# Linux-cpp-lisp/sitator

Measured on AMD Instinct MI355X. Metric: landmark-vectors/sec (frames x mobile atoms), fill + site assignment, higher is better.
Workload: dtype f64; 1 GPU; C2: SCgrid(8,8,8) orthorhombic 32.0x35.2x38.4 A, S=D=512 (V=8), M=64, A=576 (BASELINE configs[1]), 100000 frames per GPU; frames_per_gpu=100000, n_mobile=64, n_static=512, landmark_dim=512, parallelism=frame-sharded x1

## Files before the change

scratch/phase_times.py:

```python
import os, sys
sys.path.insert(0, os.path.dirname(os.path.dirname(os.path.abspath(__file__))))
os.environ["SITATOR_FILL_AUTOTUNE"] = "0"
import numpy as np
from tests.test_gpu_kernels import _setup
from sitator_amd import synth
cfg = sys.argv[1] if len(sys.argv) > 1 else "C2"
F = int(sys.argv[2]) if len(sys.argv) > 2 else 100000
host = synth.config_host(cfg)
ctx, *_ = _setup(host, synth.CONFIG_MOBILE[cfg], F, seed=2)
for _ in range(30):
    ctx.fill(check_for_zeros=False)
out = {}
for mode in (11, 10, 12):
    os.environ["SITATOR_DEBUG_STOP"] = str(mode)
    for _ in range(3):
        rc, nz, err = ctx.fill(check_for_zeros=False)
    out[mode] = ctx.info()["census"]
    print("mode", mode, "fill ms %.4f" % ctx.timers()["fill"], out[mode])
os.environ.pop("SITATOR_DEBUG_STOP")
nw = out[11][3]
names = {10: ["start -> barrier A passed", "A -> barrier B passed (phase 1b)", "B -> window set-up done", "D0 passes"],
         11: ["D1 + E passes", "T + end of window", "whole wave", None],
         12: ["start -> frame requested, at barrier A", "wait at barrier A", "phase 1b work", "wait at barrier B"]}
print("waves %d; shader-clock cycles per wave (s_memtime, 100 MHz ticks x clock ratio = cycles as the SQ counts them):" % nw)
for mode in (10, 11, 12):
    for n, v in zip(names[mode], out[mode]):
        if n:
            print("  %-44s %9.0f" % (n, v / nw))
```

sitator_amd/csrc/fill3.hip:

```cpp
#include <cmath>
#include <cstdio>
#include <cstdlib>
#include <mutex>
#include <vector>
#include <algorithm>
#include <cstring>

#include "sit_internal.h"
#include "fill3_plan.h"

struct Fill3Args {
    const uint4 *vh;
    const uint4 *vh16;
    const unsigned char *nvtab;
    const uint4 *pack;
    const i32 *p_off, *f_off;
    const i32 *lattice_map;
    i32 *row_nnz, *row_idx;
    double *row_val;
    i64 N;
    int D, W;
    int pG0, pG1, pG2, fG0, fG1, fG2;
    unsigned f_base;
    int check_zeros;
    double midpoint, steepness;
    u64 *err, *scal;
    i64 frame0;
    double cen[3];
    double x0lo, x0hi;
    int nv_uniform;
    u64 *dbgbuf;
    const i32 *static_idx, *mobile_idx;
    const double *frame_dmax;
    int s0, m0, frame_mod;
    double delta2, thr2_lo, thr2_hi, static_thr;
    int store;
    const i32 *col_ptr, *col_k;
    const double *col_val;
    i64 *labels;
    double *confs;
    i32 *wlist;
    unsigned *wcount;
    i64 seg_cap;
    int nseg, normed;
    double threshold;
};

struct Fill3Head {
    Pbc P;
    const double *frames;
    const double *ref_static;
    const double *exptab;
    i64 F, A, fbeg;
    int S, M, fpb, contig, debug_stop, rcap, iw, has_fallback, tt, mcap, prio;
    int skipw;
    int lay[12];
    double safe2;
};
typedef const Fill3Args __attribute__((address_space(4))) *Fill3ArgsPtr;


__device__ __forceinline__ double sqrt_nr(double x)
{
    const double y = __builtin_amdgcn_rsq(x);
    const double g = x * y, h = 0.5 * y;
    const double r = __builtin_fma(-h, g, 0.5);
    return __builtin_fma(g, r, g);
}

__device__ __forceinline__ double rcp_nr(double b)
{
    double y = __builtin_amdgcn_rcp(b);
    double e = __builtin_fma(-b, y, 1.0);
    y = __builtin_fma(y, e, y);
    e = __builtin_fma(-b, y, 1.0);
    return __builtin_fma(y, e, y);
}

struct ExpK {
    double log2e_128, magic, ln2_128, c4, c3, smid;
};
__device__ __forceinline__ double in_vgpr(double x) { asm volatile("" : "+v"(x)); return x; }
__device__ __forceinline__ double max_f64(double x, double c)
{
    double r;
    asm("v_max_f64 %0, %1, %2" : "=v"(r) : "v"(x), "s"(c));
    return r;
}
__device__ __forceinline__ ExpK expk_make(double mid, double steep)
{
    ExpK k;
    k.log2e_128 = in_vgpr(0x1.71547652b82fep+7);
    k.magic = in_vgpr(6755399441055744.0);
    k.ln2_128 = in_vgpr(0x1.62e42fefa39efp-8);
    k.c4 = in_vgpr(1.0 / 24); k.c3 = in_vgpr(1.0 / 6);
    k.smid = in_vgpr(steep * mid);
    return k;
}

__device__ __forceinline__ double exp_tab(double x, const double *tab, const ExpK &k)
{
    x = max_f64(x, -700.0);
    double u;
    asm("v_fma_f64 %0, %1, %2, %3" : "=v"(u) : "v"(x), "v"(k.log2e_128), "v"(k.magic));
    const double n = u - k.magic;
    const int ni = (int)(unsigned)__double_as_longlong(u);
    const double r = __builtin_fma(-n, k.ln2_128, x);
    double q = __builtin_fma(r, k.c4, k.c3);
    q = __builtin_fma(r, q, 0.5);
// ... 79 lines not shown

#define F3_LANES(m) __builtin_amdgcn_inverse_ballot_w64(m)

__device__ __forceinline__ unsigned long long first_lanes(int n)
{
    return n >= 64 ? ~0ull : ((1ull << n) - 1ull);
}

template <int CELL>
__device__ __forceinline__ void wrapc3(const Pbc &P, double &x, double &y, double &z)
{
    if (CELL == 1) {
        double b0 = P.ci[0] * x; b0 -= floor(b0);
        double b1 = P.ci[4] * y; b1 -= floor(b1);
        double b2 = P.ci[8] * z; b2 -= floor(b2);
        x = P.cm[0] * b0; y = P.cm[4] * b1; z = P.cm[8] * b2;
    } else {
        wrap3(P, x, y, z);
    }
}

template <int CELL>
__device__ __forceinline__ int bin_of3(const Pbc &P, double px, double py, double pz, int G0, int G1, int G2)
{
    double f0, f1, f2;
    if (CELL == 1) { f0 = P.ci[0] * px; f1 = P.ci[4] * py; f2 = P.ci[8] * pz; }
    else {
        f0 = (P.ci[0] * px + P.ci[1] * py + P.ci[2] * pz);
        f1 = (P.ci[3] * px + P.ci[4] * py + P.ci[5] * pz);
        f2 = (P.ci[6] * px + P.ci[7] * py + P.ci[8] * pz);
    }
    f0 -= floor(f0); f1 -= floor(f1); f2 -= floor(f2);
    int b0 = (int)(f0 * G0), b1 = (int)(f1 * G1), b2 = (int)(f2 * G2);
    b0 = b0 < 0 ? 0 : (b0 >= G0 ? G0 - 1 : b0);
    b1 = b1 < 0 ? 0 : (b1 >= G1 ? G1 - 1 : b1);
    b2 = b2 < 0 ? 0 : (b2 >= G2 ? G2 - 1 : b2);
    return (b0 * G1 + b1) * G2 + b2;
}

#define F3_TASK_OFFSETS(TK, R0X, R0Y, VOFF, IONOFF, STATOFF, FLX)                                                          \
    do {                                                                                                                   \
        VOFF = (R0X); STATOFF = 0u; FLX = 0u;                                                                              \
        const unsigned ion_ = (TK) & ~KMASK;                                                                               \
        if (FPB1) {                                                                                                        \
            IONOFF = mad24_24(ion_, ionbase);                                                                              \
            if (DYN) VOFF = 24u * (unsigned)g.lattice_map[f0 * S + (i64)(R0Y)];                                            \
        } else {                                                                                                           \
            const uint4 ir = ((const uint4 *)ionrec)[ion_];                                                                \
            IONOFF = ir.y; STATOFF = ir.z; FLX = ir.w;                                                                     \
            if (DYN) VOFF = 24u * (unsigned)g.lattice_map[(f0 + (i64)ir.w) * S + (i64)(R0Y)];                              \
        }                                                                                                                  \
    } while (0)

#define F3_D0_PASSES(NP0)                                                                                                   \
    do {                                                                                                                    \
        uint4 en_[NP0];                                                                                                     \
        unsigned ionoff_[NP0], statoff_[NP0], tfl_[NP0];                                                                    \
        int ion_[NP0];                                                                                                      \
        unsigned long long vmask_[NP0];                                                                                     \
        uint2 ii_[NP0];                                                                                                     \
        bool in_[NP0];                                                                                                      \
        if (SLOT) {                                                                                                         \
             \
             \
                                            \
            _Pragma("unroll") for (int u = 0; u < NP0; u++) {                                                               \
                ion_[u] = base + d0_step * u + s_ion;                                                                       \
                in_[u] = ion_[u] < nib;                                                                                     \
                ii_[u] = ioninfo[ib0 + ion_[u]];                                                                            \
                ionoff_[u] = ionbase + 24u * (unsigned)(base + d0_step * u) + s_ioff;                                       \
            }                                                                                                               \
                     \
            _Pragma("unroll") for (int u = 0; u < NP0; u++) asm volatile("" : "+v"(ii_[u].x), "+v"(ii_[u].y));              \
        }                                                                                                                   \
        _Pragma("unroll") for (int u = 0; u < NP0; u++) {                                                                   \
            statoff_[u] = 0u; tfl_[u] = 0u;                                                                                 \
            if (SLOT) {                                                                                                     \
                 \
                 \
                const bool act_ = in_[u] && s_slot < (int)(ii_[u].y & 255u);                                                \
                vmask_[u] = __ballot(act_);                                                                                 \
                en_[u] = pack[act_ ? ii_[u].x + (unsigned)s_slot : 0u];                                                     \
            } else {                                                                                                        \
                en_[u] = make_uint4(0u, 0u, 0u, 0x7ff00000u);       \
                const int b_ = base + 64 * u, t = b_ + lane;                                                                \
                vmask_[u] = first_lanes(nlt0 - b_);                                                                         \
                const uint2 mw = *(const uint2 *)(mark + (b_ >> 5));                        \
                const unsigned m_lo = (unsigned)__builtin_amdgcn_readfirstlane((int)mw.x), m_hi = (unsigned)__builtin_amdgcn_readfirstlane((int)mw.y); \
                const unsigned rk = __builtin_amdgcn_mbcnt_hi(m_hi, __builtin_amdgcn_mbcnt_lo(m_lo, (unsigned)carry));      \
                carry += __builtin_popcount(m_lo) + __builtin_popcount(m_hi);                                               \
                if (FPB1) {                                                                                                 \
                    const uint2 rr = ((const uint2 *)ionrec)[rk];                                                           \
                    ion_[u] = (int)rr.y;                                                                                    \
                    if (F3_LANES(vmask_[u])) en_[u] = pack[rr.x + (unsigned)t];                                             \
                    ionoff_[u] = ionbase + 24u * (unsigned)ion_[u];                                                         \
                } else {                                                                                                    \
                    ion_[u] = (int)rk2ion[rk];                                                                              \
                    const uint4 ir = ((const uint4 *)ionrec)[ion_[u]];                                                      \
                    if (F3_LANES(vmask_[u])) en_[u] = pack[ir.x + (unsigned)t];                                             \
                    ionoff_[u] = ir.y; statoff_[u] = ir.z; tfl_[u] = ir.w;                                                  \
                }                                                                                                           \
            }                                                                                                               \
        }                                                                                                                   \
              \
        if (SLOT) { _Pragma("unroll") for (int u = 0; u < NP0; u++) asm volatile("" : "+v"(en_[u].x)); }                    \
        _Pragma("unroll") for (int u = 0; u < NP0; u++) {                                                                  \
            const uint4 en = en_[u];                                                                                       \
            unsigned voff = en.y;                                                                                          \
            if (DYN) voff = 24u * (unsigned)g.lattice_map[(f0 + (i64)tfl_[u]) * S + (i64)(en.y / 24u)];                    \
            const double hk = __hiloint2double((int)en.w, (int)en.z);                                                      \
            const double *sp = lds_f64(statoff_[u] + voff);                                                                \
            const double *op = lds_f64(ionoff_[u]);                                                                        \
            double qx = sp[0] + op[0], qy = sp[1] + op[1], qz = sp[2] + op[2];                                             \
            double d2;                                                                                                     \
            if (CHEAP) {                                                                                                   \
                       \
                                                           \
                qx = minimg1(qx, P.ci[0], P.cm[0]); qy = minimg1(qy, P.ci[4], P.cm[4]); qz = minimg1(qz, P.ci[8], P.cm[8]); \
                d2 = __builtin_fma(qz, qz, __builtin_fma(qy, qy, qx * qx));                                                \
            } else {                                                                                                       \
                wrapc3<CELL>(P, qx, qy, qz);                                                                               \
                const double dx = qx - P.cen[0], dy = qy - P.cen[1], dz = qz - P.cen[2];                                   \
                d2 = (dx * dx + dy * dy) + dz * dz;                                                                        \
            }                                                                                                              \
            const unsigned long long km = __ballot(!(d2 > hk)) & vmask_[u];                                                \
            if (F3_LANES(km)) ttab[mask_rank(km, t_end)] = (en.x & KMASK) | (unsigned)ion_[u];                             \
            t_end += __popcll(km);                                                                                         \
        }                                                                                                                  \
    } while (0)

#define F3_D1E_LOAD(NP, C0, TK, R0, CLAMP)                                                                                 \
    do {                                                                                                                   \
        _Pragma("unroll") for (int u = 0; u < NP; u++) {                                                                   \
            int tb_ = TPP * ((C0) + u);                                                                                    \
            if (CLAMP) tb_ = tb_ < TT - TPP ? tb_ : TT - TPP;                                           \
// ... 158 lines not shown
        if (act && !wsp && n >= 1 && n <= 4) {                                                                             \
            i32 d0 = (i32)(svq[0] >> KSH), d1 = 0, d2 = 0, d3 = 0;                                                         \
            double v0 = pq[0], v1 = 0.0, v2 = 0.0, v3 = 0.0;                                                               \
            if (n > 1) { d1 = (i32)(svq[1] >> KSH); v1 = pq[1]; }                                                          \
            if (n > 2) { d2 = (i32)(svq[2] >> KSH); v2 = pq[2]; }                                                          \
            if (n > 3) { d3 = (i32)(svq[3] >> KSH); v3 = pq[3]; }                                                          \
            double x2 = 0.0;                                                                                               \
            x2 += v0 * v0;                                                                                                 \
            if (n > 1) x2 += v1 * v1;                                                                                      \
            if (n > 2) x2 += v2 * v2;                                                                                      \
            if (n > 3) x2 += v3 * v3;                                                                                      \
            const double xn = sqrt(x2);                                                                                    \
            const Best b = merge4_row(n, d0, d1, d2, d3, v0, v1, v2, v3, xn, g.normed != 0, g.col_ptr, g.col_k, g.col_val); \
            i64 to;                                                                                                        \
            double conf;                                                                                                   \
            finish_assignment(b, g.threshold, to, conf);                                                                   \
            g.labels[row] = to;                                                                                            \
            g.confs[row] = conf;                                                                                           \
        }                                                                                                                  \
        if (act && !wsp && n > 4 && !g.store) {                                                                            \
            for (int e = 0; e < n; e++) {                                                                                  \
                if (e < g.W) { g.row_idx[(i64)e * g.N + row] = (i32)(svq[e] >> KSH); g.row_val[(i64)e * g.N + row] = pq[e]; } \
                else atomicAdd(&g.scal[3], 1ull);                                                                          \
            }                                                                                                              \
            g.row_nnz[row] = n < g.W ? n : g.W;                                                                            \
        }                                                                                                                  \
        const bool listed = act && n >= 1 && (wsp || n > 4);                                                               \
        if (__ballot(listed)) {                                                                                            \
            const i64 sg = (i64)(blockIdx.x % (unsigned)g.nseg);                                                           \
            list_rows_by_class(listed && n <= 8, listed && n > 8, row, g.wlist + sg * g.seg_cap, g.wcount + 2 * sg,        \
                               g.seg_cap, lane);                                                                           \
        }                                                                                                                  \
    } while (0)

template <int N>
__device__ __forceinline__ double dpp_row_shl(double x)
{
    const int lo = __double2loint(x), hi = __double2hiint(x);
    return __hiloint2double(__builtin_amdgcn_mov_dpp(hi, 0x100 + N, 0xf, 0xf, true),
                            __builtin_amdgcn_mov_dpp(lo, 0x100 + N, 0xf, 0xf, true));
}

#define F3_STAMP(var) do { if (DBG == 2 && dbg >= 10) var = __builtin_amdgcn_s_memtime(); } while (0)
#define F3_SPAN(mode, word, t0, t1) do { if (DBG == 2 && dbg == (mode) && lane == 0) atomicAdd(&g.dbgbuf[4 * (blockIdx.x & 1023u) + (word)], (u64)((t1) - (t0))); } while (0)

#ifndef F3_WPE
#define F3_WPE 7
#endif
#if F3_WPE > 0
#define F3_WPE_ATTR __attribute__((amdgpu_waves_per_eu(NW == 16 ? 8 : F3_WPE, NW == 16 ? 8 : F3_WPE)))
#else
#define F3_WPE_ATTR
#endif
template <int CELL, int LG, int NW, int DYN, int FPB1, int DBG, int FUSE, int SLOT = 0>
__global__ __launch_bounds__(NW * 64) F3_WPE_ATTR void k_fill3(Fill3Head h, Fill3ArgsPtr full)
{
    static_assert(!SLOT || FPB1, "the slot form is for one frame per workgroup");
    constexpr int VP = 1 << LG;
    constexpr bool CHEAP = CELL == 1;
    constexpr int NT = NW * 64;
    constexpr int TPP = 64 >> LG;
    constexpr int KSH = CELL == 1 ? LG + 4 : LG + 5;
    constexpr int RSH = KSH - LG;
    constexpr unsigned KMASK = ~((1u << KSH) - 1u);
    constexpr unsigned long long LEADS = LG == 4 ? 0x0001000100010001ull : (LG == 3 ? 0x0101010101010101ull : 0x1111111111111111ull);
    extern __shared__ __attribute__((aligned(16))) char smem[];
    const int S = h.S, M = h.M, SM = S + M;
    const int fpb = FPB1 ? 1 : h.fpb;
    const int tid = threadIdx.x, lane = tid & 63, wave = __builtin_amdgcn_readfirstlane(tid >> 6);
    const int rcap = h.rcap, IW = h.iw, TT = h.tt;
    const int dbg = DBG ? h.debug_stop : 0;
    F3Layout L;
    L.fmax = h.lay[0]; L.gsync = h.lay[1]; L.ioninfo = h.lay[2]; L.etab = h.lay[3]; L.wave0 = h.lay[4]; L.o_ionrec = h.lay[5];
    L.o_ttab = h.lay[6]; L.o_sv = h.lay[7]; L.o_nzc = h.lay[8]; L.o_mark = h.lay[9]; L.wbytes = h.lay[10]; L.total = h.lay[11];
    double *xyz = (double *)smem;
    u64 *fmax = (u64 *)(smem + L.fmax);
    unsigned *wflag = (unsigned *)(fmax + fpb);
    unsigned *garrive = (unsigned *)(smem + L.gsync);
    unsigned *wspill = garrive + NW;
    uint2 *ioninfo = (uint2 *)(smem + L.ioninfo);
    double *etab = (double *)(smem + L.etab);
    char *wp = smem + L.wave0 + wave * L.wbytes;
    double *prod = (double *)wp;
    unsigned *ionrec = (unsigned *)(wp + L.o_ionrec);
    unsigned *ttab = (unsigned *)(wp + L.o_ttab);
    unsigned *sv = (unsigned *)(wp + L.o_sv);
    unsigned *nzc = (unsigned *)(wp + L.o_nzc);
    unsigned *mark = (unsigned *)(wp + L.o_mark);
    unsigned char *rk2ion = (unsigned char *)(wp + L.o_ionrec) + 16 * IW;
    const Pbc &P = h.P;
    const i64 f0 = h.fbeg + (i64)blockIdx.x * fpb;
    const int nf = FPB1 ? 1 : (int)((h.F - f0) < fpb ? (h.F - f0) : fpb);
    const u64 errw = (u64)(S + 1 + M);
    const Fill3Args __attribute__((address_space(4))) &g = *full;

    if ((unsigned)(size_t)(__attribute__((address_space(3))) char *)smem != 0u) {
        if (tid == 0) atomicMin(g.err, 0ull);
        return;
    }
    unsigned long long ts0 = 0, ts1 = 0, ts2 = 0, ts3 = 0, ts4 = 0, tsa = 0, tsb = 0, acc_d0 = 0, acc_d1 = 0;
    F3_STAMP(ts0);
    const int prio1 = h.prio & 3;
    if (prio1) f3_setprio(prio1);
    if (tid < fpb) fmax[tid] = 0ull;
    if (CHEAP && !DYN) for (int q = tid; q < 2 * ((fpb * S + 63) / 64); q += NT) wflag[q] = 0u;
    if (FUSE && tid < 2 * NW) garrive[tid] = 0u;
    double etv = 0.0;
    if (tid < F3_EXPN) etv = h.exptab[tid];
    for (int q = lane; q < TT; q += 64) ttab[q] = 0u;
    if (!SLOT) for (int q = lane; q < (FPB1 ? 2 * (IW + 1) : 4 * IW + (IW + 4) / 4); q += 64) ionrec[q] = 0u;
    {
        const double *fbase = h.frames + (g.frame_mod > 0 ? f0 % g.frame_mod : f0) * h.A * 3;
        if (h.contig == 4) {
            const int n2 = (nf * SM * 3 + 1) >> 1;
            const char *src = (const char *)fbase;
            for (int e0 = wave * 64; e0 < n2; e0 += NT) {
                if (e0 + lane < n2)
                    __builtin_amdgcn_global_load_lds((const __attribute__((address_space(1))) void *)(src + 16 * (size_t)(e0 + lane)),
                                                     (__attribute__((address_space(3))) void *)(smem + 16 * e0), 16, 0, 2);
            }
        } else if (h.contig == 3) {
            const int n2 = (nf * SM * 3) >> 1;
            const double2 *src2 = (const double2 *)fbase;
            double2 *dst2 = (double2 *)xyz;
            for (int e0 = tid; e0 < n2; e0 += 4 * NT) {
                double2 v[4];
#pragma unroll
                for (int u = 0; u < 4; u++) { const int e = e0 + u * NT; v[u] = e < n2 ? src2[e] : make_double2(0.0, 0.0); }
#pragma unroll
                for (int u = 0; u < 4; u++) { const int e = e0 + u * NT; if (e < n2) dst2[e] = v[u]; }
            }
        } else if (h.contig == 2) {
            const int n = nf * SM * 3;
            for (int e0 = tid; e0 < n; e0 += 8 * NT) {
                double v[8];
#pragma unroll
                for (int u = 0; u < 8; u++) { const int e = e0 + u * NT; v[u] = e < n ? fbase[e] : 0.0; }
#pragma unroll
                for (int u = 0; u < 8; u++) { const int e = e0 + u * NT; if (e < n) xyz[e] = v[u]; }
            }
        } else {
            for (int fl = 0; fl < nf; fl++) {
                const double *src = fbase + (i64)fl * h.A * 3;
                double *dst = xyz + 3 * fl * SM;
                const int n = 3 * SM;
                for (int e0 = tid; e0 < n; e0 += 8 * NT) {
                    double v[8];
#pragma unroll
                    for (int u = 0; u < 8; u++) {
                        const int e = e0 + u * NT;
                        v[u] = 0.0;
                        if (e < n) {
                            if (h.contig == 1) v[u] = src[e < 3 * S ? 3 * g.s0 + e : 3 * g.m0 + (e - 3 * S)];
                            else { const int a = e / 3; v[u] = src[3 * (a < S ? g.static_idx[a] : g.mobile_idx[a - S]) + (e - 3 * a)]; }
                        }
                    }
#pragma unroll
                    for (int u = 0; u < 8; u++) { const int e = e0 + u * NT; if (e < n) dst[e] = v[u]; }
                }
            }
        }
    }
    if (tid < F3_EXPN) etab[tid] = etv;
    F3_STAMP(tsa);
    __syncthreads();
    F3_STAMP(ts1);
    F3_SPAN(10, 0, ts0, ts1); F3_SPAN(12, 0, ts0, tsa); F3_SPAN(12, 1, tsa, ts1);
    const bool skipw = CHEAP && !DYN && h.skipw != 0;
    for (int a = tid; a < nf * SM; a += NT) {
        int fl = 0;
        if (!FPB1) for (int q = 1; q < nf; q++) fl += a >= q * SM;
        const int r = a - fl * SM;
        double *d = xyz + 3 * a;
        double x = d[0], y = d[1], z = d[2];
        if (r < S) {
            bool need_store = !skipw;
            if (!skipw) wrapc3<CELL>(P, x, y, z);
            if (!DYN) {
                const double rx = h.ref_static[r], ry = h.ref_static[S + r], rz_ = h.ref_static[2 * S + r];
                const double ex = x - rx, ey = y - ry, ez = z - rz_;
                const double e2 = (ex * ex + ey * ey) + ez * ez;
                if (!(e2 <= h.safe2)) {
                    if (skipw) {
                        wrapc3<CELL>(P, x, y, z);
                        need_store = true;
                        atomicOr(&wflag[(fl * S + r) >> 5], 1u << ((fl * S + r) & 31));
                    }
                    const double c0 = CHEAP ? g.cen[0] : P.cen[0], c1 = CHEAP ? g.cen[1] : P.cen[1], c2 = CHEAP ? g.cen[2] : P.cen[2];
                    double qx = x + (c0 - rx), qy = y + (c1 - ry), qz = z + (c2 - rz_);
                    wrapc3<CELL>(P, qx, qy, qz);
                    const double dx = -qx + c0, dy = -qy + c1, dz = -qz + c2;
                    const double d2 = (dx * dx + dy * dy) + dz * dz;
                    if (d2 > g.delta2) {
                        atomicOr(&fmax[fl], 1ull);
                        if (d2 > g.thr2_lo && (d2 > g.thr2_hi || sqrt(d2) > g.static_thr))
                            atomicMin(g.err, (u64)(g.frame0 + f0 + fl) * errw + (u64)r);
                    }
                }
            }
            if (need_store) { d[0] = x; d[1] = y; d[2] = z; }
        } else {
            wrapc3<CELL>(P, x, y, z);
            if (CHEAP) { d[0] = -x; d[1] = -y; d[2] = -z; }
            else { d[0] = P.cen[0] - x; d[1] = P.cen[1] - y; d[2] = P.cen[2] - z; }
            const int b = bin_of3<CELL>(P, x, y, z, g.pG0, g.pG1, g.pG2);
            i32 lo, hi;
            { uint2 pr; __builtin_memcpy(&pr, g.p_off + b, 8); lo = (i32)pr.x; hi = (i32)pr.y; }
            if (SLOT && hi - lo > 8) atomicMax((unsigned *)fmax + 2 * fl + 1, (unsigned)(hi - lo));
            unsigned fb = 0u;
            if (h.has_fallback) fb = (unsigned)bin_of3<CELL>(P, x, y, z, g.fG0, g.fG1, g.fG2);
            ioninfo[fl * M + (r - S)] = make_uint2((unsigned)lo, (unsigned)(hi - lo) | (fb << 8));
        }
    }
    F3_STAMP(tsb);
    __syncthreads();
    F3_STAMP(ts2);
    F3_SPAN(10, 1, ts1, ts2); F3_SPAN(12, 2, ts1, tsb); F3_SPAN(12, 3, tsb, ts2);
    bool frame_tight = true;
    int lgsl_frame = 3;
    if (SLOT) {
        const uint2 fm = *(const uint2 *)fmax;
        const unsigned beyond = (unsigned)__builtin_amdgcn_readfirstlane((int)fm.x), lmax = (unsigned)__builtin_amdgcn_readfirstlane((int)fm.y);
        if (h.has_fallback) frame_tight = DYN ? (g.frame_dmax[f0] * g.frame_dmax[f0] <= g.delta2) : beyond == 0u;
        lgsl_frame = 3 + (lmax > 8u) + (lmax > 16u) + (lmax > 32u) + (lmax > 64u);
    }
    if (SLOT) {
        if (tid == 0 && !frame_tight) atomicAdd(&g.scal[2], 1ull);
    } else if (tid < nf && h.has_fallback) {
        const bool tight = DYN ? (g.frame_dmax[f0 + tid] * g.frame_dmax[f0 + tid] <= g.delta2) : (fmax[tid] == 0ull);
        if (!tight) atomicAdd(&g.scal[2], 1ull);
    }
    if (dbg == 1) return;
    if (prio1) __builtin_amdgcn_s_setprio(0);

    const char *vh = CHEAP ? (const char *)g.vh16 : (const char *)g.vh;
    const uint4 *pack = g.pack;
    const ExpK ek = expk_make(g.midpoint, g.steepness);
    const double x0lo = g.x0lo;
    const int nvu = g.nv_uniform;
    const int hh = lane & (VP - 1), gi = lane >> LG;
    const unsigned hh32 = (unsigned)hh << RSH;
    const unsigned long long ltmask = (1ull << lane) - 1ull;
    const unsigned xyz_s = 24u * (unsigned)S;
    const int GW = FUSE ? (IW <= 32 ? 64 / IW : 1) : 1;
    constexpr bool PF = NW < 16 && FPB1 && !DBG;
    unsigned tkn_[2] = {0u, 0u};
    uint4 rn_[2] = {make_uint4(0u, 0u, 0u, 0u), make_uint4(0u, 0u, 0u, 0u)};

    const int nions = nf * M;
    bool spilled = false;
    for (int ib0 = wave * IW; ib0 < nions; ib0 += NW * IW) {
        const int nib = (nions - ib0) < IW ? (nions - ib0) : IW;
        int fl = 0, j = 0, nL = 0;
        unsigned lo = 0u;
        int nlt = 0, lgsl = 0;
        if (SLOT) {
            lgsl = lgsl_frame;
            if (lane < nib) { j = ib0 + lane; nzc[lane] = 0u; }
            if (h.has_fallback && !frame_tight) {
                if (lane < nib) {
                    const unsigned fb = ioninfo[ib0 + lane].y >> 8;
                    uint2 pr;
                    __builtin_memcpy(&pr, g.f_off + fb, 8);
                    nL = (int)(pr.y - pr.x);
                    ioninfo[ib0 + lane] = make_uint2(g.f_base + pr.x, (unsigned)nL | (fb << 8));
                }
                lgsl = 3 + (__ballot(nL > 8) != 0ull) + (__ballot(nL > 16) != 0ull) + (__ballot(nL > 32) != 0ull) + (__ballot(nL > 64) != 0ull);
            }
            if (lgsl > 6) { if (lane == 0) atomicAdd(&g.scal[3], 1ull); break; }
        } else {
            if (lane < nib) {
                const int ion = ib0 + lane;
                if (!FPB1) for (int q = 1; q < nf; q++) fl += ion >= q * M;
                j = ion - fl * M;
                const uint2 ii = ioninfo[ion];
                lo = ii.x; nL = (int)(ii.y & 255u);
                if (h.has_fallback) {
                    const bool tight = DYN ? (g.frame_dmax[f0 + fl] * g.frame_dmax[f0 + fl] <= g.delta2) : (fmax[fl] == 0ull);
                    if (!tight) {
                        const unsigned fb = ii.y >> 8;
                        uint2 pr;
                        __builtin_memcpy(&pr, g.f_off + fb, 8);
                        nL = (int)(pr.y - pr.x); lo = g.f_base + pr.x;
                    }
                }
            }
            const int inL = wave_add_scan(nL), exL = inL - nL;
            nlt = __builtin_amdgcn_readlane(inL, 63);
            if (nlt > h.mcap) { if (lane == 0) atomicAdd(&g.scal[3], 1ull); break; }
            for (int q = lane; q < 2 * ((nlt + 63) >> 6); q += 64) mark[q] = 0u;
            {
                const unsigned long long nem = __ballot(nL > 0);
                if (lane < nib) {
                    if (nL > 0) {
                        const int rk = mask_rank(nem, 0);
                        atomicOr(&mark[(inL - 1) >> 5], 1u << ((inL - 1) & 31));
                        if (FPB1) ((uint2 *)ionrec)[rk] = make_uint2(lo - (unsigned)exL, (unsigned)lane);
                        else rk2ion[rk] = (unsigned char)lane;
                    }
                    if (!FPB1) ((uint4 *)ionrec)[lane] = make_uint4(lo - (unsigned)exL, 24u * (unsigned)(fl * SM + S + j), 24u * (unsigned)(fl * SM), (unsigned)fl);
                    nzc[lane] = 0u;
                }
            }
        }
        if (DBG && dbg == 9 && lane == 0) { atomicAdd(&g.scal[5], (u64)nlt); atomicAdd(&g.scal[7], 1ull); }
        const unsigned ionbase = xyz_s + 24u * (unsigned)ib0;
        F3_STAMP(ts3);
        F3_SPAN(10, 2, ts2, ts3);
        int t_end = 0, carry = 0, cnt = 0;
        spilled = false;
        const int nlt0 = (DBG && dbg == 2) ? 0 : nlt;
        const int d0_lim = SLOT ? ((DBG && dbg == 2) ? 0 : nib) : nlt0, d0_step = SLOT ? 64 >> lgsl : 64;
        const int s_ion = lane >> lgsl, s_slot = lane & ((1 << lgsl) - 1);
        const unsigned s_ioff = 24u * (unsigned)s_ion;
        for (int base = 0; base < d0_lim; base += d0_step) {
            F3_STAMP(ts4);
            if (NW < 16 && base + d0_step < d0_lim && t_end <= TT - 128) { F3_D0_PASSES(2); base += d0_step; }
            else F3_D0_PASSES(1);
            if (DBG == 2 && dbg >= 10) { unsigned long long tq = __builtin_amdgcn_s_memtime(); acc_d0 += tq - ts4; ts4 = tq; }
            if (t_end <= TT - 64 && base + d0_step < d0_lim) continue;
            if (DBG && dbg == 9 && lane == 0) atomicAdd(&g.scal[4], (u64)t_end);
            if (DBG && dbg == 3) t_end = 0;
            const int pend = (t_end + TPP - 1) / TPP;
            int cursor = 0;
            if (PF && pend > 0) F3_D1E_LOAD(2, 0, tkn_, rn_, false);
            while (cursor < pend) {
                while (cursor < pend && cnt + TPP <= rcap) {
                    if (cursor + 1 < pend && cnt + 2 * TPP <= rcap) {
                        F3_D1E_PASSES(2);
                        cursor += 2;
                    } else {
                        F3_D1E_PASSES(1);
                        cursor += 1;
                    }
                }
                if (DBG && dbg == 9 && lane == 0) atomicAdd(&g.scal[6], (u64)cnt);
                if (cursor < pend) F3_T_ROUND(0);
            }
            t_end = 0;
            if (DBG == 2 && dbg >= 10) { unsigned long long tq = __builtin_amdgcn_s_memtime(); acc_d1 += tq - ts4; }
        }
        if (DBG && dbg == 5) cnt = 0;
        F3_STAMP(ts4);
        F3_T_ROUND(1);
        if (lane < nib) {
            int nnz = (int)nzc[lane];
            if (FUSE && !spilled) nnz &= 255;
            if (DBG && dbg >= 2 && dbg <= 5) nnz = 1;
            const i64 row = (f0 + fl) * M + j;
            if (!FUSE || spilled || g.store) g.row_nnz[row] = nnz < g.W ? nnz : g.W;
            if (nnz == 0) {
                if (g.check_zeros) atomicMin(g.err, (u64)(g.frame0 + f0 + fl) * errw + (u64)(S + 1 + j));
                else atomicAdd(&g.scal[0], 1ull);
            }
        }
        if (DBG == 2 && dbg >= 10) {
            unsigned long long te = __builtin_amdgcn_s_memtime();
            F3_SPAN(10, 3, 0ull, acc_d0); F3_SPAN(11, 0, 0ull, acc_d1); F3_SPAN(11, 1, ts4, te); F3_SPAN(11, 2, ts0, te); F3_SPAN(11, 3, 0ull, 1ull);
        }
    }
    if (FUSE) {
        const int grp = wave / GW, gw0 = grp * GW;
        const int gsize = (NW - gw0) < GW ? (NW - gw0) : GW;
        bool mine = true;
        if (GW > 1) {
            if (lane == 0) wspill[wave] = spilled ? 1u : 0u;
            __builtin_amdgcn_fence(__ATOMIC_RELEASE, "workgroup");
            unsigned arrived = 0u;
            if (lane == 0) arrived = __hip_atomic_fetch_add(&garrive[grp], 1u, __ATOMIC_RELAXED, __HIP_MEMORY_SCOPE_WORKGROUP);
            arrived = (unsigned)__builtin_amdgcn_readfirstlane((int)arrived);
            mine = (int)arrived + 1 == gsize;
// ... 210 lines not shown
#undef F3_PICK
#undef F3_PICK3
#undef F3_LAUNCH
    return hipGetLastError();
}

#define F3_ARGS_BYTES 1024
#define F3_TRIAL_WORDS 17

int fill3_prepare(sit_ctx *c)
{
    int rc = fill3_basis_tables(c);
    if (rc) return rc;
    if (!c->d_fill_args) {
        if ((rc = dev_alloc(c, &c->d_fill_args, (i64)(2 * F3_ARGS_BYTES + F3_TRIAL_WORDS * 8)))) return rc;
        c->fill_args_host.clear();
    }
    return SIT_OK;
}

static int f3_fill_args(sit_ctx *c, const sit_fill_params *p, const F3PlanIn &in, const F3Plan &plan, const F3Knobs &knobs, Fill3Args *ap, Fill3Head *hp)
{
    Fill3Args &a = *ap;
    Fill3Head &h = *hp;
    const bool have_tight = in.have_tight;
    memset(&a, 0, sizeof(a));
    a.vh = (const uint4 *)c->d_vh; a.vh16 = (const uint4 *)c->d_vh16; a.nvtab = c->d_nv;
    a.pack = (const uint4 *)c->d_pack;
    a.f_off = c->d_bin_off; a.fG0 = c->G[0]; a.fG1 = c->G[1]; a.fG2 = c->G[2];
    a.f_base = (unsigned)c->pack_nt;
    if (have_tight) { a.p_off = c->d_tbin_off; a.pG0 = c->tG[0]; a.pG1 = c->tG[1]; a.pG2 = c->tG[2]; }
    else { a.p_off = c->d_bin_off; a.pG0 = c->G[0]; a.pG1 = c->G[1]; a.pG2 = c->G[2]; }
    a.lattice_map = in.dynmap ? c->d_lattice_map : nullptr;
    a.row_nnz = c->d_row_nnz; a.row_idx = c->d_row_idx;
    a.N = c->N; a.D = (int)c->D; a.W = (int)c->rows_W;
    a.check_zeros = p->check_for_zeros;
    a.midpoint = c->midpoint; a.steepness = c->steepness;
    a.x0lo = c->f3_x0lo; a.x0hi = c->f3_x0hi;
    a.err = c->d_err; a.scal = c->d_scal; a.frame0 = c->frame0;
    for (int i = 0; i < 3; i++) a.cen[i] = c->pbc.cen[i];
    if (knobs.force_exact) { a.x0lo = -INFINITY; a.x0hi = INFINITY; }
    a.nv_uniform = knobs.nvu ? c->nv_uniform : 0;
    a.frame_mod = knobs.frame_mod;

    memset(&h, 0, sizeof(h));
    h.P = c->pbc; h.frames = c->d_frames; a.static_idx = c->d_static_idx; a.mobile_idx = c->d_mobile_idx;
    h.ref_static = c->d_ref_soa;
    a.frame_dmax = in.dynmap ? c->d_frame_dmax : nullptr;
    h.exptab = c->d_exptab;
    h.F = in.f_hi; h.fbeg = in.f_lo; h.A = c->A;
    h.S = (int)in.S; h.M = (int)in.M;
    h.debug_stop = f3_debug_stop(knobs, in.dynmap);
    h.has_fallback = have_tight ? 1 : 0;
    a.s0 = (int)c->idx_s0; a.m0 = (int)c->idx_m0;
    a.delta2 = have_tight ? c->tight_delta * c->tight_delta : -1.0;
    a.thr2_lo = c->static_thr * c->static_thr * (1.0 - 1e-14);
    a.thr2_hi = c->static_thr * c->static_thr * (1.0 + 1e-14);
    a.static_thr = c->static_thr;
    {
        double safe = 0.45 * c->hmin;
        if (have_tight && c->tight_delta < safe) safe = c->tight_delta;
        if (c->static_thr * (1.0 - 1e-9) < safe) safe = c->static_thr * (1.0 - 1e-9);
        h.safe2 = safe > 0 ? safe * safe * (1.0 - 1e-12) : -1.0;
    }
    a.row_val = plan.fuse || plan.store ? c->d_row_val : nullptr;
    a.store = plan.store ? 1 : 0;
    int rc;
    if (plan.fuse) {
        const i64 grid_all = (i64)(unsigned)((in.f_hi - in.f_lo + plan.fpb - 1) / plan.fpb);
        const int nseg = (int)std::min<i64>(grid_all > 0 ? grid_all : 1, (i64)cu_count(c) * 4);
        const i64 seg_cap = (grid_all + nseg - 1) / nseg * ((i64)plan.fpb * in.M);
        if ((rc = wide_list_carve(c, nseg, seg_cap, &a.wcount, &a.wlist))) return rc;
        a.seg_cap = seg_cap; a.nseg = nseg;
        a.col_ptr = c->d_col_ptr; a.col_k = c->d_col_k; a.col_val = c->d_col_val;
        a.labels = c->d_labels; a.confs = c->d_confs;
        a.normed = c->centers_normed; a.threshold = p->predict_threshold;
    }
    if (h.debug_stop >= 10) {
        if ((rc = ensure_scratch(c, 1024 * 4 * 8 + 64))) return rc;
        a.dbgbuf = (u64 *)c->d_scratch;
        HIP_TRY(c, hipMemsetAsync(a.dbgbuf, 0, 1024 * 4 * 8, c->stream));
    }
    if (c->fill_args_host.size() != sizeof(Fill3Args) || memcmp(c->fill_args_host.data(), &a, sizeof(Fill3Args)) != 0) {
        c->fill_args_host.assign((const char *)&a, (const char *)&a + sizeof(Fill3Args));
        HIP_TRY(c, hipMemcpyAsync(c->d_fill_args, c->fill_args_host.data(), sizeof(Fill3Args), hipMemcpyHostToDevice, c->stream));
    }
    return SIT_OK;
}

struct F3Tuned { i64 key[8]; int rcap, tt; };
static std::mutex g_f3_mutex;
static std::vector<F3Tuned> g_f3_tuned;

static int f3_autotune(sit_ctx *c, const F3PlanIn &in, const F3Knobs &knobs, const Fill3Args &a, const Fill3Head &h, F3Plan *plan)
{
    const i64 key[8] = {in.S, in.M, c->D, in.vp, in.have_tight ? in.W_tight : in.W, (i64)plan->nw * 64 + plan->fpb, in.dynmap ? 1 : 0,
                        (i64)(c->tight_mean_candidates * 4.0 + 0.5)};
    {
        std::lock_guard<std::mutex> lock(g_f3_mutex);
        for (const F3Tuned &t : g_f3_tuned) if (memcmp(t.key, key, sizeof(key)) == 0) { *plan = f3_plan_with(*plan, t.rcap, t.tt); return SIT_OK; }
    }
    struct Ev { hipEvent_t e = nullptr; ~Ev() { if (e) (void)hipEventDestroy(e); } } ev0, ev1;
    HIP_TRY(c, hipEventCreate(&ev0.e)); HIP_TRY(c, hipEventCreate(&ev1.e));
    Fill3Head ht = h;
    Fill3Args at = a;
    at.err = (u64 *)(c->d_fill_args + 2 * F3_ARGS_BYTES); at.scal = at.err + 1;
// ... 84 lines not shown
```

Measured before the change: 9.558 billion lvec/s.

## Issue frame loads before prelude and prefetch first D0 pass loads early

Moves the shared-memory initialisation prelude after the frame-load request so the global frame fetch is in flight sooner, and passes frame_mod through kernel arguments. It peels each thread's mobile-ion bin lookup ahead of the static loop so the p_off load latency overlaps other work. It also hoists the first wave's ioninfo and pack loads and the first D0 pass ahead of the window loop, overlapping them with barrier and set-up work. The cost is more live registers and more complex control flow, which could lower occupancy.

```diff
diff --git a/scratch/phase_times.py b/scratch/phase_times.py
--- a/scratch/phase_times.py
+++ b/scratch/phase_times.py
@@ -11,7 +11,7 @@
 for _ in range(30):
     ctx.fill(check_for_zeros=False)
 out = {}
-for mode in (11, 10, 12):
+for mode in (11, 10, 12, 13):
     os.environ["SITATOR_DEBUG_STOP"] = str(mode)
     for _ in range(3):
         rc, nz, err = ctx.fill(check_for_zeros=False)
@@ -21,9 +21,10 @@
 nw = out[11][3]
 names = {10: ["start -> barrier A passed", "A -> barrier B passed (phase 1b)", "B -> window set-up done", "D0 passes"],
          11: ["D1 + E passes", "T + end of window", "whole wave", None],
-         12: ["start -> frame requested, at barrier A", "wait at barrier A", "phase 1b work", "wait at barrier B"]}
+         12: ["start -> frame requested, at barrier A", "wait at barrier A", "phase 1b work", "wait at barrier B"],
+         13: ["start -> frame requested (no wait for it)", "requested -> at barrier A (frame landed)", None, None]}
 print("waves %d; shader-clock cycles per wave (s_memtime, 100 MHz ticks x clock ratio = cycles as the SQ counts them):" % nw)
-for mode in (10, 11, 12):
+for mode in (10, 11, 12, 13):
     for n, v in zip(names[mode], out[mode]):
         if n:
             print("  %-44s %9.0f" % (n, v / nw))
diff --git a/sitator_amd/csrc/fill3.hip b/sitator_amd/csrc/fill3.hip
--- a/sitator_amd/csrc/fill3.hip
+++ b/sitator_amd/csrc/fill3.hip
@@ -55,6 +55,7 @@
     int S, M, fpb, contig, debug_stop, rcap, iw, has_fallback, tt, mcap, prio;
     int skipw;
     int lay[12];
+    int frame_mod;
     double safe2;
 };
 typedef const Fill3Args __attribute__((address_space(4))) *Fill3ArgsPtr;
@@ -240,7 +241,7 @@
         }                                                                                                                  \
     } while (0)
 
-#define F3_D0_PASSES(NP0)                                                                                                   \
+#define F3_D0_PASSES(NP0, PRE)                                                                                              \
     do {                                                                                                                    \
         uint4 en_[NP0];                                                                                                     \
         unsigned ionoff_[NP0], statoff_[NP0], tfl_[NP0];                                                                    \
@@ -255,11 +256,11 @@
             _Pragma("unroll") for (int u = 0; u < NP0; u++) {                                                               \
                 ion_[u] = base + d0_step * u + s_ion;                                                                       \
                 in_[u] = ion_[u] < nib;                                                                                     \
-                ii_[u] = ioninfo[ib0 + ion_[u]];                                                                            \
+                ii_[u] = (PRE) ? pre_ii[u] : ioninfo[ib0 + ion_[u]];                                                        \
                 ionoff_[u] = ionbase + 24u * (unsigned)(base + d0_step * u) + s_ioff;                                       \
             }                                                                                                               \
                      \
-            _Pragma("unroll") for (int u = 0; u < NP0; u++) asm volatile("" : "+v"(ii_[u].x), "+v"(ii_[u].y));              \
+            if (!(PRE)) { _Pragma("unroll") for (int u = 0; u < NP0; u++) asm volatile("" : "+v"(ii_[u].x), "+v"(ii_[u].y)); } \
         }                                                                                                                   \
         _Pragma("unroll") for (int u = 0; u < NP0; u++) {                                                                   \
             statoff_[u] = 0u; tfl_[u] = 0u;                                                                                 \
@@ -268,7 +269,7 @@
                  \
                 const bool act_ = in_[u] && s_slot < (int)(ii_[u].y & 255u);                                                \
                 vmask_[u] = __ballot(act_);                                                                                 \
-                en_[u] = pack[act_ ? ii_[u].x + (unsigned)s_slot : 0u];                                                     \
+                en_[u] = (PRE) ? pre_en[u] : pack[act_ ? ii_[u].x + (unsigned)s_slot : 0u];                                 \
             } else {                                                                                                        \
                 en_[u] = make_uint4(0u, 0u, 0u, 0x7ff00000u);       \
                 const int b_ = base + 64 * u, t = b_ + lane;                                                                \
@@ -533,6 +534,9 @@
 #else
 #define F3_WPE_ATTR
 #endif
+#ifndef F3_EARLY_LOADS
+#define F3_EARLY_LOADS 7
+#endif
 template <int CELL, int LG, int NW, int DYN, int FPB1, int DBG, int FUSE, int SLOT = 0>
 __global__ __launch_bounds__(NW * 64) F3_WPE_ATTR void k_fill3(Fill3Head h, Fill3ArgsPtr full)
 {
@@ -575,23 +579,32 @@
     const u64 errw = (u64)(S + 1 + M);
     const Fill3Args __attribute__((address_space(4))) &g = *full;
 
-    if ((unsigned)(size_t)(__attribute__((address_space(3))) char *)smem != 0u) {
-        if (tid == 0) atomicMin(g.err, 0ull);
-        return;
-    }
-    unsigned long long ts0 = 0, ts1 = 0, ts2 = 0, ts3 = 0, ts4 = 0, tsa = 0, tsb = 0, acc_d0 = 0, acc_d1 = 0;
+    constexpr bool EARLY_A = (F3_EARLY_LOADS & 1) != 0;
+    constexpr bool EARLY_B = (F3_EARLY_LOADS & 2) != 0 && FPB1 && NW < 16;
+    constexpr bool EARLY_C = (F3_EARLY_LOADS & 4) != 0 && SLOT && NW < 16;
+    unsigned long long ts0 = 0, ts1 = 0, ts2 = 0, ts3 = 0, ts4 = 0, tsa = 0, tsb = 0, tsr = 0, acc_d0 = 0, acc_d1 = 0;
     F3_STAMP(ts0);
     const int prio1 = h.prio & 3;
+    if (EARLY_A) asm volatile("" : : "s"(h.S), "s"(h.M), "s"(h.contig), "s"(h.frame_mod));
+    double etv = 0.0;
+#define F3_PRELUDE()                                                                                                       \
+    do {                                                                                                                   \
+        if ((unsigned)(size_t)(__attribute__((address_space(3))) char *)smem != 0u) {       \
+            if (tid == 0) atomicMin(g.err, 0ull);                                                                          \
+            return;                                                                                                        \
+        }                                                                                                                  \
+        if (tid < fpb) fmax[tid] = 0ull;                                                                                   \
+        if (CHEAP && !DYN) for (int q = tid; q < 2 * ((fpb * S + 63) / 64); q += NT) wflag[q] = 0u;                        \
+        if (FUSE && tid < 2 * NW) garrive[tid] = 0u;                                                                       \
+        if (tid < F3_EXPN) etv = h.exptab[tid];                        \
+        for (int q = lane; q < TT; q += 64) ttab[q] = 0u;           \
+        if (!SLOT) for (int q = lane; q < (FPB1 ? 2 * (IW + 1) : 4 * IW + (IW + 4) / 4); q += 64) ionrec[q] = 0u;       \
+    } while (0)
     if (prio1) f3_setprio(prio1);
-    if (tid < fpb) fmax[tid] = 0ull;
-    if (CHEAP && !DYN) for (int q = tid; q < 2 * ((fpb * S + 63) / 64); q += NT) wflag[q] = 0u;
-    if (FUSE && tid < 2 * NW) garrive[tid] = 0u;
-    double etv = 0.0;
-    if (tid < F3_EXPN) etv = h.exptab[tid];
-    for (int q = lane; q < TT; q += 64) ttab[q] = 0u;
-    if (!SLOT) for (int q = lane; q < (FPB1 ? 2 * (IW + 1) : 4 * IW + (IW + 4) / 4); q += 64) ionrec[q] = 0u;
+    if (!EARLY_A) F3_PRELUDE();
     {
-        const double *fbase = h.frames + (g.frame_mod > 0 ? f0 % g.frame_mod : f0) * h.A * 3;
+        const int fmod = EARLY_A ? h.frame_mod : g.frame_mod;
+        const double *fbase = h.frames + (fmod > 0 ? f0 % fmod : f0) * h.A * 3;
         if (h.contig == 4) {
             const int n2 = (nf * SM * 3 + 1) >> 1;
             const char *src = (const char *)fbase;
@@ -642,13 +655,46 @@
             }
         }
     }
+    F3_STAMP(tsr);
+    if (EARLY_A) F3_PRELUDE();
+#undef F3_PRELUDE
     if (tid < F3_EXPN) etab[tid] = etv;
     F3_STAMP(tsa);
     __syncthreads();
     F3_STAMP(ts1);
-    F3_SPAN(10, 0, ts0, ts1); F3_SPAN(12, 0, ts0, tsa); F3_SPAN(12, 1, tsa, ts1);
+    F3_SPAN(10, 0, ts0, ts1); F3_SPAN(12, 0, ts0, tsa); F3_SPAN(12, 1, tsa, ts1); F3_SPAN(13, 0, ts0, tsr); F3_SPAN(13, 1, tsr, tsa);
     const bool skipw = CHEAP && !DYN && h.skipw != 0;
-    for (int a = tid; a < nf * SM; a += NT) {
+#define F3_ION_REQUEST(D_, X, Y, Z, PR, FB)                                                                                \
+    do {                                                                                                                   \
+        wrapc3<CELL>(P, X, Y, Z);                                                                                          \
+        if (CHEAP) { (D_)[0] = -X; (D_)[1] = -Y; (D_)[2] = -Z; }                                                           \
+        else { (D_)[0] = P.cen[0] - X; (D_)[1] = P.cen[1] - Y; (D_)[2] = P.cen[2] - Z; }                                   \
+                \
+                                                   \
+        const int b = bin_of3<CELL>(P, X, Y, Z, g.pG0, g.pG1, g.pG2);                                                      \
+        __builtin_memcpy(&PR, g.p_off + b, 8);                          \
+        FB = 0u;                                                                                                           \
+        if (h.has_fallback) FB = (unsigned)bin_of3<CELL>(P, X, Y, Z, g.fG0, g.fG1, g.fG2);                                 \
+    } while (0)
+#define F3_ION_RECORD(FL, J, PR, FB)                                                                                       \
+    do {                                                                                                                   \
+        const i32 lo = (i32)PR.x, hi = (i32)PR.y;                                                                          \
+            \
+                                       \
+        if (SLOT && hi - lo > 8) atomicMax((unsigned *)fmax + 2 * (FL) + 1, (unsigned)(hi - lo));                          \
+        ioninfo[(FL) * M + (J)] = make_uint2((unsigned)lo, (unsigned)(hi - lo) | (FB << 8));                               \
+    } while (0)
+    const bool peel = EARLY_B && M <= NT;
+    const int mj = (tid - S) & (NT - 1);
+    const bool peel_mine = peel && mj < M;
+    uint2 ppr = make_uint2(0u, 0u);
+    unsigned pfb = 0u;
+    if (peel_mine) {
+        double *d = xyz + 3 * (S + mj);
+        double x = d[0], y = d[1], z = d[2];
+        F3_ION_REQUEST(d, x, y, z, ppr, pfb);
+    }
+    for (int a = tid; a < (peel ? S : nf * SM); a += NT) {
         int fl = 0;
         if (!FPB1) for (int q = 1; q < nf; q++) fl += a >= q * SM;
         const int r = a - fl * SM;
@@ -681,18 +727,15 @@
             }
             if (need_store) { d[0] = x; d[1] = y; d[2] = z; }
         } else {
-            wrapc3<CELL>(P, x, y, z);
-            if (CHEAP) { d[0] = -x; d[1] = -y; d[2] = -z; }
-            else { d[0] = P.cen[0] - x; d[1] = P.cen[1] - y; d[2] = P.cen[2] - z; }
-            const int b = bin_of3<CELL>(P, x, y, z, g.pG0, g.pG1, g.pG2);
-            i32 lo, hi;
-            { uint2 pr; __builtin_memcpy(&pr, g.p_off + b, 8); lo = (i32)pr.x; hi = (i32)pr.y; }
-            if (SLOT && hi - lo > 8) atomicMax((unsigned *)fmax + 2 * fl + 1, (unsigned)(hi - lo));
-            unsigned fb = 0u;
-            if (h.has_fallback) fb = (unsigned)bin_of3<CELL>(P, x, y, z, g.fG0, g.fG1, g.fG2);
-            ioninfo[fl * M + (r - S)] = make_uint2((unsigned)lo, (unsigned)(hi - lo) | (fb << 8));
+            uint2 pr;
+            unsigned fb;
+            F3_ION_REQUEST(d, x, y, z, pr, fb);
+            F3_ION_RECORD(fl, r - S, pr, fb);
         }
     }
+    if (peel_mine) F3_ION_RECORD(0, mj, ppr, pfb);
+#undef F3_ION_REQUEST
+#undef F3_ION_RECORD
     F3_STAMP(tsb);
     __syncthreads();
     F3_STAMP(ts2);
@@ -704,6 +747,20 @@
         const unsigned beyond = (unsigned)__builtin_amdgcn_readfirstlane((int)fm.x), lmax = (unsigned)__builtin_amdgcn_readfirstlane((int)fm.y);
         if (h.has_fallback) frame_tight = DYN ? (g.frame_dmax[f0] * g.frame_dmax[f0] <= g.delta2) : beyond == 0u;
         lgsl_frame = 3 + (lmax > 8u) + (lmax > 16u) + (lmax > 32u) + (lmax > 64u);
+    }
+    uint2 pre_ii[2] = {make_uint2(0u, 0u), make_uint2(0u, 0u)};
+    uint4 pre_en[2] = {make_uint4(0u, 0u, 0u, 0u), make_uint4(0u, 0u, 0u, 0u)};
+    if (EARLY_C) {
+        const int nib1 = (M - wave * IW) < IW ? (M - wave * IW) : IW;
+        const int ib1 = nib1 > 0 ? wave * IW : 0;
+#pragma unroll
+        for (int u = 0; u < 2; u++) pre_ii[u] = ioninfo[ib1 + 8 * u + (lane >> 3)];
+        asm volatile("" : "+v"(pre_ii[0].x), "+v"(pre_ii[0].y), "+v"(pre_ii[1].x), "+v"(pre_ii[1].y));
+#pragma unroll
+        for (int u = 0; u < 2; u++) {
+            const bool act = 8 * u + (lane >> 3) < nib1 && (lane & 7) < (int)(pre_ii[u].y & 255u);
+            pre_en[u] = g.pack[act ? pre_ii[u].x + (unsigned)(lane & 7) : 0u];
+        }
     }
     if (SLOT) {
         if (tid == 0 && !frame_tight) atomicAdd(&g.scal[2], 1ull);
@@ -730,6 +787,23 @@
 
     const int nions = nf * M;
     bool spilled = false;
+    int pre_adv = -1, pre_tend = 0;
+    unsigned long long pre_clk = 0;
+    if (EARLY_C && wave * IW < nions && lgsl_frame == 3 && !(h.has_fallback && !frame_tight)) {
+        const int ib0 = wave * IW, nib = (nions - ib0) < IW ? (nions - ib0) : IW;
+        const unsigned ionbase = xyz_s + 24u * (unsigned)ib0;
+        const int d0_lim = (DBG && dbg == 2) ? 0 : nib, d0_step = 8, base = 0, nlt0 = 0;
+        const int s_ion = lane >> 3, s_slot = lane & 7;
+        const unsigned s_ioff = 24u * (unsigned)s_ion;
+        int t_end = 0, carry = 0;
+        F3_STAMP(ts4);
+        if (d0_lim > 0) {
+            if (d0_step < d0_lim && TT >= 128) { F3_D0_PASSES(2, 1); pre_adv = d0_step; }
+            else { F3_D0_PASSES(1, 1); pre_adv = 0; }
+        }
+        pre_tend = t_end;
+        if (DBG == 2 && dbg >= 10) { pre_clk = __builtin_amdgcn_s_memtime() - ts4; acc_d0 += pre_clk; }
+    }
     for (int ib0 = wave * IW; ib0 < nions; ib0 += NW * IW) {
         const int nib = (nions - ib0) < IW ? (nions - ib0) : IW;
         int fl = 0, j = 0, nL = 0;
@@ -787,8 +861,9 @@
         if (DBG && dbg == 9 && lane == 0) { atomicAdd(&g.scal[5], (u64)nlt); atomicAdd(&g.scal[7], 1ull); }
         const unsigned ionbase = xyz_s + 24u * (unsigned)ib0;
         F3_STAMP(ts3);
-        F3_SPAN(10, 2, ts2, ts3);
-        int t_end = 0, carry = 0, cnt = 0;
+        F3_SPAN(10, 2, ts2 + pre_clk, ts3);
+        int t_end = EARLY_C ? pre_tend : 0, carry = 0, cnt = 0;
+        pre_tend = 0;
         spilled = false;
         const int nlt0 = (DBG && dbg == 2) ? 0 : nlt;
         const int d0_lim = SLOT ? ((DBG && dbg == 2) ? 0 : nib) : nlt0, d0_step = SLOT ? 64 >> lgsl : 64;
@@ -796,8 +871,9 @@
         const unsigned s_ioff = 24u * (unsigned)s_ion;
         for (int base = 0; base < d0_lim; base += d0_step) {
             F3_STAMP(ts4);
-            if (NW < 16 && base + d0_step < d0_lim && t_end <= TT - 128) { F3_D0_PASSES(2); base += d0_step; }
-            else F3_D0_PASSES(1);
+            if (EARLY_C && pre_adv >= 0) { base += pre_adv; pre_adv = -1; }
+            else if (NW < 16 && base + d0_step < d0_lim && t_end <= TT - 128) { F3_D0_PASSES(2, 0); base += d0_step; }
+            else F3_D0_PASSES(1, 0);
             if (DBG == 2 && dbg >= 10) { unsigned long long tq = __builtin_amdgcn_s_memtime(); acc_d0 += tq - ts4; ts4 = tq; }
             if (t_end <= TT - 64 && base + d0_step < d0_lim) continue;
             if (DBG && dbg == 9 && lane == 0) atomicAdd(&g.scal[4], (u64)t_end);
@@ -1114,6 +1190,7 @@
     h.S = (int)in.S; h.M = (int)in.M;
     h.debug_stop = f3_debug_stop(knobs, in.dynmap);
     h.has_fallback = have_tight ? 1 : 0;
+    h.frame_mod = knobs.frame_mod;
     a.s0 = (int)c->idx_s0; a.m0 = (int)c->idx_m0;
     a.delta2 = have_tight ? c->tight_delta * c->tight_delta : -1.0;
     a.thr2_lo = c->static_thr * c->static_thr * (1.0 - 1e-14);
```

After: 9.638 billion lvec/s, median of 6. No clear change (+0.8%).
